# UbiquitousLearning/Mandheling-DSP-Training

Hardware: AMD Instinct MI355X
Metric: training images/sec + int8 MFMA TOPS, VGG-11 batch 256, 1/2/4/8 MI355X (higher is better)
Workload: dtype int8; 1 GPU; VGG11 NITI int8 training step (fwd+relu+pool, loss grad, weight grad, input grad, SGD), 3x32x32; global_batch=256, per_gpu_batch=256, parallelism=single GPU, streams=one stream (weight gradient, then input gradient, per layer)

## Files before the change

include/niti_hip.h:

```cpp
#ifndef NITI_HIP_H
#define NITI_HIP_H

#include <stddef.h>
#include <stdint.h>

#ifdef __cplusplus
extern "C" {
#endif

enum niti_error_code {
    NITI_NO_ERROR = 0,
    NITI_OUT_OF_MEMORY = 1,
    NITI_NOT_SUPPORT = 2,
    NITI_COMPUTE_SIZE_ERROR = 3,
    NITI_NO_EXECUTION = 4,
    NITI_INVALID_VALUE = 5,
    NITI_INPUT_DATA_ERROR = 10,
    NITI_CALL_BACK_STOP = 11
};

enum niti_op_type {
    NITI_OP_CONV_INT8 = 700,
    NITI_OP_DECONV_INT8 = 701,
    NITI_OP_RELU_INT8 = 703,
// ... 85 lines not shown
int niti_conv_fwd_phase1(const niti_geom* g, const int8_t* x_nhwc16, const int8_t* w_ohwi16, int32_t* acc,
                         uint32_t* amax, void* workspace, size_t workspace_bytes, void* stream);
int niti_conv_fwd_phase2(const niti_geom* g, const int8_t* x_nhwc16, const int8_t* w_ohwi16, const int32_t* acc,
                         const uint32_t* amax, const int8_t* exp_in, const int8_t* wscale, int8_t* exp_out, int relu,
                         const int8_t* relu_mask, int8_t* out_nhwc16, size_t workspace_bytes, void* stream);
int niti_conv_dgrad_phase1(const niti_geom* g, const int8_t* dy_nhwc16, const int8_t* wt_ihwo16, int32_t* acc,
                           uint32_t* amax, void* workspace, size_t workspace_bytes, void* stream);
int niti_conv_dgrad_phase2(const niti_geom* g, const int8_t* dy_nhwc16, const int8_t* wt_ihwo16, const int32_t* acc,
                           const uint32_t* amax, const int8_t* exp_in, const int8_t* wscale, int8_t* exp_out,
                           int relu, const int8_t* relu_mask, int8_t* out_nhwc16, size_t workspace_bytes,
                           void* stream);
#define NITI_ROWCONV_STATE_WORDS 1216
uint32_t* niti_rows_spec_slot(uint32_t* state, int dgrad);
int niti_conv_rows_ok(const niti_geom* g);
int niti_conv_rows_plan(const niti_geom* g, int dgrad, int* W, int* R, int* ks, int* workgroups);
int niti_nhwc16_to_c32(const int8_t* in_nhwc16, int n, int hw, int cp, int c, int8_t* out_c32, void* stream);
int niti_weights_to_wf(const int8_t* w_ohwi16, int co, int ci, int cip, int transpose, int8_t* out_wf,
                       void* stream);
#define NITI_ROWS_X_NHWC16 0x100
int niti_conv_rows_nhwc_ok(const niti_geom* g, int flags);
int niti_conv_fwd_rows(const niti_geom* g, const int8_t* x_c32, const int8_t* wf, const int8_t* exp_in,
                       const int8_t* wscale, int8_t* exp_out, int relu, int8_t* out_nhwc16, int8_t* pool_out_nhwc16,
                       int8_t* next_c32, int mode, uint32_t* amax, uint32_t* state, uint32_t epoch, uint32_t* err,
                       void* stream);
int niti_conv_dgrad_rows(const niti_geom* g, const int8_t* dy_c32, const int8_t* wft, const int8_t* relu_mask,
                         const int8_t* pool_x, const int8_t* pool_y, int pool_relu, int8_t* dx_nhwc16, int8_t* dx_c32,
                         int8_t* dx_p16, const int8_t* exp_in, const int8_t* wscale, int8_t* exp_out, int mode,
                         uint32_t* amax, uint32_t* state, uint32_t epoch, uint32_t* err, void* stream);
int niti_conv_wgrad_acc(const niti_geom* g, const int8_t* x_nhwc16, const int8_t* dy_nhwc16, int32_t* acc,
                        uint32_t* amax, void* workspace, size_t workspace_bytes, void* stream);
int niti_nhwc16_to_p16(const int8_t* in_nhwc16, int64_t pixels, int cp, int8_t* out_p16, void* stream);
int niti_conv_wgrad_p16_workspace(const niti_geom* g, int splits, size_t* bytes);
void niti_diag_wgrad_stamps(void* buf);
void niti_diag_rowconv_stamps(void* buf);
void niti_diag_rowconv_barrier(uint32_t spin_limit, uint32_t expect_extra);
void niti_diag_rowconv_speculate(int mode);
void niti_diag_gemm_speculate(int bias);
unsigned long long niti_diag_gemm_fused_launches(void);
unsigned long long niti_diag_head_chain_launches(void);
void niti_diag_head_chain(int on);
void niti_diag_p16_jobs_cap(int cap);
int niti_conv_wgrad_p16_acc(const niti_geom* g, const int8_t* x_p16, const int8_t* dy_p16, int32_t* acc,
                            uint32_t* amax, void* workspace, size_t workspace_bytes, int splits, void* stream);
typedef struct niti_wgrad_p16_job {
    niti_geom g;
    const int8_t* x_p16;
    const int8_t* dy_p16;
    int32_t* acc;
    uint32_t* amax;
} niti_wgrad_p16_job;
int niti_conv_wgrad_p16_many_workspace(const niti_wgrad_p16_job* jobs, int n, int blocks, int t, size_t* bytes);
// ... 282 lines not shown
```

mandheling-dsp-training_amd/csrc/niti_capi.hip:

```cpp
#include "../../include/niti_hip.h"
#include <memory>
#include <vector>

#include "niti_internal.hpp"
#include "niti_kernels.hpp"

struct niti_execution {
    niti::Execution* impl = nullptr;
    int op = 0;
    std::vector<void*> stage;
    std::vector<size_t> stage_bytes;
    uint32_t* err_host = nullptr;
    ~niti_execution() {
        delete impl;
        for (void* p : stage)
            if (p) (void)hipFree(p);
        if (err_host) (void)hipHostFree(err_host);
    }
};

namespace {
int code(hipError_t e) {
    if (e == hipSuccess) return NITI_NO_ERROR;
    if (e == hipErrorOutOfMemory) return NITI_OUT_OF_MEMORY;
// ... 258 lines not shown
    o.exp_in = exp_in;
    o.wscale = wscale;
    o.exp_out = exp_out;
    return o;
}

int niti_conv_rows_ok(const niti_geom* g) {
    niti::ConvGeom r;
    return g && to_geom(g, &r) && niti::rowconv_ok(r) ? 1 : 0;
}

int niti_conv_rows_plan(const niti_geom* g, int dgrad, int* W, int* R, int* ks, int* workgroups) {
    niti::ConvGeom r, d;
    if (!g || !W || !R || !ks || !workgroups || !to_geom(g, &r)) return 0;
    if (dgrad && !niti::rowconv_dgrad_geom(r, &d)) return 0;
    return niti::rowconv_plan(dgrad ? d : r, dgrad != 0, W, R, ks, workgroups) ? 1 : 0;
}

int niti_nhwc16_to_c32(const int8_t* in, int n, int hw, int cp, int c, int8_t* out, void* stream) {
    if (!in || !out || n <= 0 || hw <= 0 || c <= 0 || cp < c || cp % 16) return NITI_INVALID_VALUE;
    return code(niti::nhwc16_to_c32(in, n, hw, cp, c, out, S(stream)));
}

int niti_weights_to_wf(const int8_t* w, int co, int ci, int cip, int transpose, int8_t* out, void* stream) {
    if (!w || !out || co <= 0 || ci <= 0 || cip < ci || cip % 16) return NITI_INVALID_VALUE;
    return code(niti::weights_to_wf(w, co, ci, cip, transpose != 0, out, S(stream)));
}

int niti_conv_rows_nhwc_ok(const niti_geom* g, int dgrad) {
    if (!g) return 0;
    niti::ConvGeom r, d;
    if (!to_geom(g, &r)) return 0;
// ... 29 lines not shown
}

int niti_conv_dgrad_rows(const niti_geom* g, const int8_t* dy_c32, const int8_t* wft, const int8_t* relu_mask,
                         const int8_t* pool_x, const int8_t* pool_y, int pool_relu, int8_t* dx, int8_t* dx_c32,
                         int8_t* dx_p16, const int8_t* exp_in, const int8_t* wscale, int8_t* exp_out, int mode,
                         uint32_t* amax, uint32_t* state, uint32_t epoch, uint32_t* err, void* stream) {
    const int x_nhwc = (mode & NITI_ROWS_X_NHWC16) ? 1 : 0;
    mode &= ~NITI_ROWS_X_NHWC16;
    if (!g || !dy_c32 || !wft || !amax || mode < 0 || mode > 4) return NITI_INVALID_VALUE;
    if (mode >= 3 && state == nullptr) return NITI_INVALID_VALUE;
    if ((pool_x == nullptr) != (pool_y == nullptr) || (pool_x && relu_mask)) return NITI_INVALID_VALUE;
    if (mode != 1 && dx == nullptr) return NITI_INVALID_VALUE;
    niti::ConvGeom r, d;
    if (!to_geom(g, &r)) return NITI_COMPUTE_SIZE_ERROR;
    if (!niti::rowconv_dgrad_geom(r, &d)) return NITI_NOT_SUPPORT;
    if (mode == 0 && !niti::rowconv_fused_ok(d, true)) return NITI_NOT_SUPPORT;
    if (dx_p16 != nullptr && !niti::rowconv_p16_ok(d, pool_x != nullptr)) return NITI_NOT_SUPPORT;
    if (x_nhwc && !niti::rowconv_nhwc_ok(d)) return NITI_NOT_SUPPORT;
    niti::RowConvOut o;
    o.x_nhwc = x_nhwc;
    o.p16 = dx_p16;
    o.exp_in = exp_in;
    o.wscale = wscale;
    o.exp_out = exp_out;
    o.dgrad_slot = 1;
    if (pool_x != nullptr) {
        o.pool_x = pool_x;
        o.pool_y = pool_y;
        o.pool_dx = dx;
        o.pool_dx_next = dx_c32;
        o.pool_relu = pool_relu;
// ... 690 lines not shown
```

mandheling-dsp-training_amd/csrc/niti_kernels.hpp:

```cpp
#pragma once

#include <hip/hip_runtime.h>
#include <stdint.h>
#include <stdlib.h>

#include "../../include/niti_hip.h"

namespace niti {

inline int round_up(int x, int m) { return (x + m - 1) / m * m; }

constexpr int MAX_SLOTS = 64;
constexpr int MAX_SLOT_STRIDE = 32;
constexpr int MAX_WORDS = MAX_SLOTS * MAX_SLOT_STRIDE;
constexpr size_t MAX_BYTES = MAX_WORDS * sizeof(uint32_t);

struct ConvGeom {
    int n, c_in, h, w;
    int c_out, kh, kw;
    int sh, sw, pt, pl, pb, pr, dh, dw;
    int oh, ow;
    int cip, cop, np;
    bool finalize();
};
// ... 217 lines not shown
    int relu = 0;
    const int8_t* relu_mask = nullptr;
    const int8_t* pool_x = nullptr;
    const int8_t* pool_y = nullptr;
    int8_t* pool_dx = nullptr;
    int8_t* pool_dx_next = nullptr;
    int pool_relu = 0;
    const int8_t* pool_code = nullptr;
    int8_t* pool_code_out = nullptr;
    int pool_dx_nhwc = 1;
    int8_t* p16 = nullptr;
    int32_t* acc_store = nullptr;
    int dgrad_slot = 0;
    int x_nhwc = 0;
};
size_t rowconv_acc_bytes(const ConvGeom& g, bool dg);
bool rowconv_nhwc_ok(const ConvGeom& g);
bool rowconv_nhwc_pref(const ConvGeom& g);
constexpr int ROWCONV_BAR_WORDS = 2 * 19 * 32;
static_assert(ROWCONV_BAR_WORDS == NITI_ROWCONV_STATE_WORDS, "header constant");
bool rowconv_ok(const ConvGeom& g);
bool rowconv_seg(const ConvGeom& g);
bool rowconv_dgrad_geom(const ConvGeom& layer, ConvGeom* d);
bool rowconv_p16_ok(const ConvGeom& d, bool pool);
bool rowconv_fused_ok(const ConvGeom& g, bool dg = false);
int rowconv_units(const ConvGeom& g, bool dg = false);
bool rowconv_plan(const ConvGeom& g, bool dg, int* W, int* R, int* ks, int* wgs);
size_t rowconv_wf_bytes(int co, int ci);
hipError_t nhwc16_to_c32(const int8_t* in, int n, int hw, int cp, int c, int8_t* out, hipStream_t st);
hipError_t c32_to_nhwc16(const int8_t* in, int n, int hw, int cp, int c, int8_t* out, hipStream_t st);
hipError_t weights_to_wf(const int8_t* w_ohwi16, int co, int ci, int cip, bool transpose, int8_t* out,
                         hipStream_t st);
constexpr int RC_SPEC_A = 3, RC_SPEC_B = 4;
bool rowconv_spec2_on();
void rowconv_stamps_arm(unsigned long long* buf);
void rowconv_barrier_diag(uint32_t spin_limit, uint32_t expect_extra);
void rowconv_speculate(int mode);
uint32_t* rowconv_spec_slot(uint32_t* bar, bool dg);
void model_p16_jobs_cap(int cap);
void model_wgrad_batch(int mode);
void model_wgrad_quad(int kg);
int wgrad_quad_kg(int own);
// ... 197 lines not shown
```

mandheling-dsp-training_amd/csrc/niti_model.hip:

```cpp
#include <stdlib.h>
#include <string.h>

#include <algorithm>
#include <array>
#include <memory>
#include <vector>

#include "../../include/niti_hip.h"
#include "niti_map.hpp"
#include "niti_step_driver.hpp"

namespace niti {

namespace {
extern int g_p16_jobs_cap;
extern int g_wgrad_batch;
extern int g_wgrad_quad;
extern int g_c0w_mode;
extern unsigned long long g_c0w_launches;
}
void model_p16_jobs_cap(int cap) { g_p16_jobs_cap = cap <= 0 ? P16_MAX_JOBS : cap; }
void model_wgrad_batch(int mode) { g_wgrad_batch = mode < 0 ? 1 : mode; }
void model_wgrad_quad(int kg) { g_wgrad_quad = kg < 0 ? -1 : kg; }
int wgrad_quad_kg(int own) { return g_wgrad_quad >= 0 ? g_wgrad_quad : own; }
// ... 744 lines not shown
        }
        if (!l.col && !l.dw && rowconv_ok(g)) {
            l.rc = 1;
            l.wf = (int8_t*)ws.alloc(rowconv_wf_bytes(g.c_out, g.c_in));
            l.xc32 = (int8_t*)ws.alloc((size_t)n * round_up(g.c_in, 32) * g.h * g.w);
            if (!l.wf || !l.xc32) return NITI_OUT_OF_MEMORY;
            if (hipMemset(l.wf, 0, rowconv_wf_bytes(g.c_out, g.c_in)) != hipSuccess)
                return NITI_NO_EXECUTION;
            rc_acc_size = std::max(rc_acc_size, rowconv_acc_bytes(g, false));
            const Layer* pv = i > 0 ? &L[i - 1] : nullptr;
            const bool pv_ok = pv != nullptr && !pv->flatten && pv->g.cop == g.cip &&
                               (pv->pool ? (pv->ph == g.h && pv->pw == g.w && pv->g.oh == 2 * g.h && pv->g.ow == 2 * g.w)
                                         : (pv->g.oh == g.h && pv->g.ow == g.w));
            if (pv_ok && rowconv_dgrad_geom(g, &l.dg)) {
                l.rcd = 1;
                rc_acc_size = std::max(rc_acc_size, rowconv_acc_bytes(l.dg, true));
                l.wft = (int8_t*)ws.alloc(rowconv_wf_bytes(g.c_in, g.c_out));
                l.dyc32 = (int8_t*)ws.alloc(out_px * round_up(g.c_out, 32));
                if (!l.wft || !l.dyc32) return NITI_OUT_OF_MEMORY;
                if (hipMemset(l.wft, 0, rowconv_wf_bytes(g.c_in, g.c_out)) != hipSuccess) return NITI_NO_EXECUTION;
            }
        }
        if (!l.dw && conv_wgrad_p16_ok(g)) {
            slab_w_bytes = std::max(slab_w_bytes, conv_wgrad_p16_workspace(g, 8));
            xp16[i] = (int8_t*)ws.alloc((size_t)n * g.h * g.w * g.cip);
            l.slab16_bytes = conv_wgrad_p16_workspace(g, 8);
            l.slab16 = l.slab16_bytes ? (int32_t*)ws.alloc(l.slab16_bytes) : nullptr;
            if (l.slab16_bytes && !l.slab16) return NITI_OUT_OF_MEMORY;
            dp16[i] = (int8_t*)ws.alloc(out_px * g.cop);
            if (!xp16[i] || !dp16[i]) return NITI_OUT_OF_MEMORY;
        }
// ... 355 lines not shown
            } else {
                o.pool_x = pv.r;
                o.pool_y = pv.p;
            }
            o.pool_dx = pv.dy;
            o.pool_dx_next = next;
            o.pool_relu = pv.relu;
            o.pool_dx_nhwc = skip16 ? 0 : 1;
        } else {
            o.out = skip16 ? nullptr : pv.dy;
            o.next = next;
            o.relu_mask = pv.relu ? pv.r : nullptr;
        }
        dy16_valid[i - 1] = !skip16 && !g0_only;
        const bool dgk = !g0_only;
        const int rc = rowconv_ranged(rowconv_fused_ok(d, dgk), rowconv_acc_bytes(d, dgk) != 0, o, rng(i, 1), l.bar,
                                      l.epoch, st,
                                      [&](const RowConvOut& ro, int mode, uint32_t* bar, uint32_t epoch, uint32_t* err) {
                                          return rowconv_fwd(d, dyin, l.wft, ro, mode, rng(i, 1), bar, epoch, err, st);
                                      });
        if (rc != NITI_NO_ERROR) return rc;
        probe(i, 1, false, st);
        dp16_valid[i - 1] = o.p16 != nullptr ? 1 : 0;
        dyc32_valid[i - 1] = next != nullptr ? 1 : 0;
        return NITI_NO_ERROR;
    }
    dy16_valid[i - 1] = 1;
    const ConvGeom& pg = pv.g;
    const bool sub = l.subw != nullptr;
    const bool spec = !l.dw && conv_dgrad_spec_ok(g);
    int8_t* p16_out = !l.dw && !sub && !spec && fuse_dp16 && wgrad_p16_splits(i - 1) > 0 ? dp16[i - 1] : nullptr;
// ... 787 lines not shown
```

mandheling-dsp-training_amd/csrc/niti_rowconv.hip:

```cpp
#include <hip/hip_runtime.h>

#include <stdlib.h>

#include <algorithm>
#include <map>
#include <mutex>

#include "niti_device.hpp"
#include "niti_gridbar.hpp"
#include "niti_kernels.hpp"
#include "niti_map.hpp"

#ifndef RC_EXP
#define RC_EXP 0
#endif
namespace niti {

__device__ __forceinline__ int bitwidth_rc(uint32_t m) { return m <= 1u ? 0 : 32 - __clz((int)(m - 1u)); }

__device__ __forceinline__ int32_t psto_rc(int32_t a, int s) {
    const uint32_t ua = a < 0 ? 0u - (uint32_t)a : (uint32_t)a;
    const uint32_t q = ua >> s;
    const uint32_t prob = ua & ((1u << s) - 1u);
    const int h = s >> 1;
// ... 137 lines not shown
constexpr int RC_LDS_BYTES = RC_MAX_STAGES * RC_STAGE_BYTES;
constexpr int RC_P16_WAVE_BYTES = 16 * 1024;
constexpr int RC_SMEM_BYTES = RC_LDS_BYTES > 4 * RC_P16_WAVE_BYTES ? RC_LDS_BYTES : 4 * RC_P16_WAVE_BYTES;
constexpr int RC_KS_MAX_NS = 4;
constexpr int RC_KS_BYTES = 4 * RC_KS_MAX_NS * 9 * 1024;
static_assert(RC_KS_BYTES >= 4 * RC_P16_WAVE_BYTES, "the P16 tile fits the K-split ring");

template <int W, int R, bool UNC>
__device__ __forceinline__ void rowconv_compute(const RowConvArgs& a, const RowUnit<W, R>& U, int lane, int wid,
                                                int8_t* smem, v16i (&acc)[R]) {
    constexpr int NR = R + 2, WS = W == 0 ? 16 : W;
    const int H = W == 0 ? a.hw : W, WR = W == 0 ? a.hw : W;
    constexpr bool DPPX = true;
    constexpr int KXL = DPPX ? 1 : 3;
    constexpr int S = 4;
    constexpr int L = KXL * NR + 3;
    const int h = lane >> 5, c = lane & 31, ox = W == 0 ? U.x : c % WS;
    const __amdgpu_buffer_rsrc_t rX = make_rsrc(a.x, a.xbytes);
    const __amdgpu_buffer_rsrc_t rW = make_rsrc(a.wf, a.wbytes);
    const uint32_t xl = !(U.img_ok && U.x_ok) ? OOB
                        : W == 0 ? (uint32_t)U.img * a.xis + (uint32_t)ox * a.xps + 16u * h
                                 : (uint32_t)((((int64_t)U.img * a.CB * H) * WR + ox) * 32 + 16 * h);
    const uint32_t CHUNK = W == 0 ? a.xcs : (uint32_t)H * WR * 32;
    const uint32_t XROW = W == 0 ? a.xrs : (uint32_t)WR * 32;
    const int y0 = U.b * R - 1;
#pragma unroll
    for (int r = 0; r < R; ++r)
#pragma unroll
        for (int i = 0; i < 16; ++i) acc[r][i] = 0;
    uint32_t off[3][NR];
#pragma unroll
    for (int j = 0; j < NR; ++j) {
        const int iy = y0 + j;
        const bool row_ok = iy >= 0 && iy < H && xl != OOB;
        const uint32_t base = xl + (uint32_t)iy * XROW;
        off[0][j] = row_ok && ox > 0 ? base - 32u : OOB;
        off[1][j] = row_ok ? base : OOB;
        off[2][j] = row_ok && ox < WR - 1 ? base + 32u : OOB;
    }
    const uint32_t dv2 = wid == 0 ? (uint32_t)lane * 16u : OOB;
    const int cb = a.CB;
    constexpr bool ONE_BLOCK = W != 0;
    const uint32_t wbase =
        (uint32_t)(ONE_BLOCK ? __builtin_amdgcn_readfirstlane(U.cob * cb * 9) : U.cob * cb * 9) * 1024u;
    v4i X[S][KXL][NR];
    auto issue = [&](auto st_c, int cc) {
        constexpr int ST = decltype(st_c)::value;
        int8_t* lds = smem + ST * RC_STAGE_BYTES;
#pragma unroll
        for (int k = 0; k < 3; ++k) {
            const int piece = wid + 4 * k;
            dma16(rW, lds + piece * 1024, k < 2 ? (uint32_t)lane * 16u : dv2,
                  wbase + (uint32_t)cc * 9216u + (uint32_t)(piece < 9 ? piece : 0) * 1024u);
        }
#pragma unroll
        for (int j = 0; j < NR; ++j)
#pragma unroll
            for (int kx = 0; kx < KXL; ++kx)
                X[ST][kx][j] = buf_load16(rX, off[DPPX ? 1 : kx][j] + (uint32_t)cc * CHUNK);
    };
    const uint32_t lds_lane = lds_addr(smem) + (uint32_t)lane * 16u;
    unsigned long long t_wait = 0, t_read = 0, t_issue = 0;
    const bool stamp = a.stamps != nullptr;
    v4i wreg[2][9];
    auto read_w = [&](auto st_c, v4i (&w)[9]) {
        constexpr int ST = decltype(st_c)::value;
#pragma unroll
        for (int t = 0; t < 9; ++t) w[t] = lds_b128(lds_lane + (uint32_t)(ST * RC_STAGE_BYTES + t * 1024));
    };
    auto fence_w = [&](v4i (&w)[9]) {
        asm volatile("s_waitcnt lgkmcnt(0)" ::: "memory");
#pragma unroll
        for (int t = 0; t < 9; ++t) reg_fence(w[t]);
    };
    auto arrive = [&](int later) {
        if (later >= 1)
            asm volatile("s_waitcnt vmcnt(%0)" ::"n"(L) : "memory");
        else
            asm volatile("s_waitcnt vmcnt(0)" ::: "memory");
        __builtin_amdgcn_s_barrier();
        asm volatile("" ::: "memory");
    };
    constexpr bool SKIP = W > 0 && R == W && !(RC_EXP & 32);
// ... 13 lines not shown
            }
        if (more && !(RC_EXP & 4)) read_w(std::integral_constant<int, (ST + 1) % S>(), wreg[1 - WB]);
        const v4i (&w)[9] = wreg[(RC_EXP & 4) ? 0 : WB];
        if constexpr (DPPX) {
            v4i XL[NR], XR[NR];
            auto taps = [&](int j) {
                XL[j] = (RC_EXP & 1) ? X[ST][0][j] : shift_in_left<WS>(X[ST][0][j], ox == 0);
                XR[j] = (RC_EXP & 1) ? X[ST][0][j] : shift_in_right<WS>(X[ST][0][j], ox == WS - 1);
            };
            auto mfma3 = [&](int r, int ky) {
                acc[r] = __builtin_amdgcn_mfma_i32_32x32x32_i8(w[3 * ky], XL[r + ky], acc[r], 0, 0, 0);
                acc[r] = __builtin_amdgcn_mfma_i32_32x32x32_i8(w[3 * ky + 1], X[ST][0][r + ky], acc[r], 0, 0, 0);
                acc[r] = __builtin_amdgcn_mfma_i32_32x32x32_i8(w[3 * ky + 2], XR[r + ky], acc[r], 0, 0, 0);
            };
#pragma unroll
            for (int j = SKIP ? 1 : 0; j < (SKIP ? NR - 1 : NR); ++j) taps(j);
#pragma unroll
            for (int r = 0; r < R; ++r)
#pragma unroll
                for (int ky = SKIP && r == 0 ? 1 : 0; ky < (SKIP && r == R - 1 ? 2 : 3); ++ky) mfma3(r, ky);
        } else {
#pragma unroll
            for (int r = 0; r < R; ++r)
#pragma unroll
                for (int ky = 0; ky < 3; ++ky)
#pragma unroll
                    for (int kx = 0; kx < 3; ++kx)
                        acc[r] = __builtin_amdgcn_mfma_i32_32x32x32_i8(w[3 * ky + kx], X[ST][kx][r + ky], acc[r], 0, 0, 0);
        }
        if constexpr (ONE_BLOCK) {
            if (more) fence_w(wreg[1 - WB]);
        } else {
            const unsigned long long s2 = stamp ? __builtin_amdgcn_s_memtime() : 0ull;
            if (more) fence_w(wreg[1 - WB]);
            if (stamp) {
// ... 18 lines not shown
            step(std::integral_constant<int, 0>(), cc);
            step(std::integral_constant<int, 1>(), cc + 1);
            step(std::integral_constant<int, 2>(), cc + 2);
            step(std::integral_constant<int, 3>(), cc + 3);
        }
        asm volatile("s_waitcnt vmcnt(0)" ::: "memory");
    } else {
        for (int cc = 0; cc < cb; cc += S) {
            step(std::integral_constant<int, 0>(), cc);
            if (cc + 1 < cb) step(std::integral_constant<int, 1>(), cc + 1);
            if (cc + 2 < cb) step(std::integral_constant<int, 2>(), cc + 2);
            if (cc + 3 < cb) step(std::integral_constant<int, 3>(), cc + 3);
        }
    }
    __builtin_amdgcn_s_barrier();
    if (stamp && lane == 0) {
        unsigned long long* st = a.stamps + (blockIdx.x * 4 + wid) * 16;
        st[3] = __builtin_amdgcn_s_memtime();
        st[2] = t_issue;
        st[6] = t_wait;
        st[7] = t_read;
    }
}

template <int W, int R, int NS>
__device__ __forceinline__ void rowconv_compute_ks(const RowConvArgs& a, const RowUnit<W, R>& U, int lane, int wid,
                                                   int8_t* smem, v16i (&acc)[R]) {
    static_assert(R == W && NS >= 1 && NS <= RC_KS_MAX_NS, "whole-image units, all chunks staged at once");
    constexpr int H = W;
    const int h = lane >> 5, c = lane & 31, ox = c % W;
// ... 1076 lines not shown
    static const int v = getenv("NITI_RC_ACC_MIN_CIN") ? atoi(getenv("NITI_RC_ACC_MIN_CIN")) : 256;
    return v;
}
static bool seg_store_acc(const ConvGeom& g) { return g.c_in >= acc_min_cin(); }

bool rowconv_dgrad_geom(const ConvGeom& l, ConvGeom* d) {
    if (!rowconv_ok(l)) return false;
    ConvGeom g = l;
    g.c_in = l.c_out;
    g.c_out = l.c_in;
    if (!g.finalize() || g.cip != l.cop || g.cop != l.cip) return false;
    *d = g;
    return rowconv_ok(g);
}

static int rowconv_rows(const ConvGeom& g, bool dg, int* units_out) {
    if (rowconv_seg(g)) {
        const SegPlan p = seg_plan(g);
        *units_out = p.wgs * 4;
        return p.R;
    }
    const int W = g.w, G = 32 / W;
    const int64_t groups = (g.n + G - 1) / G, cob = g.cop / 32;
    int R = W == 16 && !dg ? 8 : (W < 4 ? W : 4);
    if (RC_EXP & 16) R = 2;
    while (R > 2 && groups * (W / R) * cob < 768) R /= 2;
    const int64_t ngb4 = (groups * (W / R) + 3) / 4 * 4;
    *units_out = (int)(ngb4 * cob);
    return R;
}

static int rowconv_ks(const ConvGeom& g, bool dg);

size_t rowconv_acc_bytes(const ConvGeom& g, bool dg) {
    if (!rowconv_ok(g)) return 0;
    if (rowconv_seg(g)) {
        const SegPlan p = seg_plan(g);
        return seg_store_acc(g) ? (size_t)p.wgs * 4 * p.R * 1024 * sizeof(int32_t) : 0;
    }
    if (getenv("NITI_RC_ACC_MIN_CIN") != nullptr && g.c_in < acc_min_cin()) return 0;
    int u = 0;
    const int R = rowconv_rows(g, dg, &u);
    const int G = 32 / g.w, ngb = ((g.n + G - 1) / G) * (g.h / R), ngb4 = (ngb + 3) / 4 * 4, COB = g.cop / 32;
    const int64_t wgs = rowconv_ks(g, dg) > 0 ? (int64_t)COB * ngb : (int64_t)COB * ngb4 / 4;
    return (size_t)wgs * 4 * R * 1024 * sizeof(int32_t);
}

bool rowconv_p16_ok(const ConvGeom& d, bool pool) {
    if (!rowconv_ok(d) || rowconv_seg(d)) return false;
    int u = 0;
    const int R = rowconv_rows(d, true, &u), W = d.w;
    const int64_t px = (int64_t)d.n * d.h * d.w * (pool ? 4 : 1);
    if (px % 16 != 0) return false;
    return pool || R * W >= 16 || (W == 2 && R == 2) || (W == 4 && R == 2);
}

static int rowconv_ks(const ConvGeom& g, bool dg) {
    int u = 0;
    const int R = rowconv_rows(g, dg, &u);
    const int CB = (g.c_in + 31) / 32;
    if (g.w != 2 || R != 2 || CB % 4 != 0 || CB / 4 > RC_KS_MAX_NS || u >= 768) return 0;
    return CB / 4;
}

int rowconv_units(const ConvGeom& g, bool dg) {
    if (rowconv_seg(g)) return seg_plan(g).wgs * 4;
    int u = 0;
    (void)rowconv_rows(g, dg, &u);
    if (rowconv_ks(g, dg) > 0) {
        const int64_t units = (int64_t)(g.n + 15) / 16 * (g.cop / 32);
        return (int)(units * 4);
    }
    return u;
}

template <int MODE, bool DG>
static const void* rc_kernel(int W, int R, bool unc, int ks) {
    if constexpr (MODE == RC_REQUANT && DG) {
        if (W == 0 && ks == 1 && R == 4) return reinterpret_cast<const void*>(&rowconv_fwd_kernel<0, 4, MODE, DG, false, 1>);
        if (W == 0 && ks == 1 && R == 2) return reinterpret_cast<const void*>(&rowconv_fwd_kernel<0, 2, MODE, DG, false, 1>);
    }
    if (W == 0 && ks != 0) return nullptr;
    if (ks > 0) {
        if (ks == 4) return reinterpret_cast<const void*>(&rowconv_fwd_kernel<2, 2, MODE, DG, false, 4>);
        if (ks == 2) return reinterpret_cast<const void*>(&rowconv_fwd_kernel<2, 2, MODE, DG, false, 2>);
        if (ks == 1) return reinterpret_cast<const void*>(&rowconv_fwd_kernel<2, 2, MODE, DG, false, 1>);
        return nullptr;
    }
#define RC_CASE(WW, RR)                                                                                  \
    if (W == WW && R == RR)                                                                              \
        return (WW != 1 && unc) ? reinterpret_cast<const void*>(&rowconv_fwd_kernel<WW, RR, MODE, DG, true, 0>) \
                                : reinterpret_cast<const void*>(&rowconv_fwd_kernel<WW, RR, MODE, DG, false, 0>);
    if constexpr (!DG) RC_CASE(16, 8)
    RC_CASE(16, 4)
    RC_CASE(16, 2)
    RC_CASE(8, 4)
    RC_CASE(8, 2)
    RC_CASE(4, 4)
    RC_CASE(4, 2)
    RC_CASE(2, 2)
    RC_CASE(1, 1)
    RC_CASE(0, 4)
    RC_CASE(0, 2)
#undef RC_CASE
    return nullptr;
}

template <int MODE, bool DG>
static hipError_t launch_rc(int W, int R, int grid, RowConvArgs a, hipStream_t st, int ks = 0) {
    const void* f = rc_kernel<MODE, DG>(W, R, W != 1 && a.CB % 4 == 0, ks);
    if (f == nullptr) return hipErrorInvalidValue;
    void* args[] = {&a};
    return hipLaunchKernel(f, dim3((unsigned)grid), dim3(256), args, 0, st);
}
// ... 7 lines not shown
        return 0;
    }
    std::lock_guard<std::mutex> lk(mu);
    const auto key = std::make_pair(dev, f);
    auto it = cache.find(key);
    if (it != cache.end()) return it->second;
    int cus = 0, occ = 0;
    if (hipDeviceGetAttribute(&cus, hipDeviceAttributeMultiprocessorCount, dev) != hipSuccess ||
        hipOccupancyMaxActiveBlocksPerMultiprocessor(&occ, f, threads, 0) != hipSuccess) {
        (void)hipGetLastError();
        return 0;
    }
    return cache[key] = cus * occ;
}

static int rowconv_wgs(const ConvGeom& g, bool dg, int* R_out, int* ks_out) {
    if (rowconv_seg(g)) {
        const SegPlan p = seg_plan(g);
        *R_out = p.R;
        *ks_out = 0;
        return p.wgs;
    }
    int u = 0;
    const int R = rowconv_rows(g, dg, &u);
    const int ks = rowconv_ks(g, dg);
    const int G = 32 / g.w, ngb = ((g.n + G - 1) / G) * (g.h / R), ngb4 = (ngb + 3) / 4 * 4, COB = g.cop / 32;
    *R_out = R;
    *ks_out = ks;
    return ks > 0 ? COB * ngb : COB * ngb4 / 4;
}

bool rowconv_plan(const ConvGeom& g, bool dg, int* W, int* R, int* ks, int* wgs) {
    if (!rowconv_ok(g)) return false;
    *wgs = rowconv_wgs(g, dg, R, ks);
    *W = rowconv_seg(g) ? 0 : g.w;
    return true;
}

bool rowconv_fused_ok(const ConvGeom& g, bool dg) {
    if (!rowconv_ok(g)) return false;
    int R = 0, ks = 0;
    const int wgs = rowconv_wgs(g, dg, &R, &ks);
    const bool unc = (g.c_in + 31) / 32 % 4 == 0;
    const int W = rowconv_seg(g) ? 0 : g.w;
    const void* f = dg ? rc_kernel<RC_FUSED, true>(W, R, unc, ks) : rc_kernel<RC_FUSED, false>(W, R, unc, ks);
    return wgs <= resident_wgs(f);
}

static uint32_t g_rc_spin_limit = BAR_SPIN_LIMIT, g_rc_expect_extra = 0;
static int g_rc_spec = 0;
void rowconv_barrier_diag(uint32_t spin_limit, uint32_t expect_extra) {
    g_rc_spin_limit = spin_limit ? spin_limit : BAR_SPIN_LIMIT;
    g_rc_expect_extra = expect_extra;
}
void rowconv_speculate(int mode) { g_rc_spec = mode; }
uint32_t* rowconv_spec_slot(uint32_t* bar, bool dg) { return bar + (16 + (dg ? 1 : 0)) * BAR_LINE; }
static bool spec_scale_on() {
// ... 48 lines not shown
        a.xcs = 32u;
    } else {
        a.xps = 32u;
        a.xrs = (uint32_t)(g.w * 32);
        a.xis = (uint32_t)(CB * g.h * g.w * 32);
        a.xcs = (uint32_t)(g.h * g.w * 32);
    }
    a.x = x_c32;
    a.wf = wf;
    a.xbytes = (uint32_t)xb;
    a.wbytes = (uint32_t)wb;
    a.n = g.n;
    a.CB = CB;
    a.COB = COB;
    const bool dg = o.relu_mask != nullptr || o.pool_dx != nullptr || o.p16 != nullptr;
    int units = 0;
    const int R = rowconv_rows(g, dg, &units);
    const bool seg = rowconv_seg(g);
    const int Wk = seg ? 0 : g.w;
    int ks = 0;
    if (seg) {
        const SegPlan p = seg_plan(g);
        a.hw = g.w;
        a.gw = p.gw;
        a.nsp = p.nsp;
        a.nbands = p.nbands;
        a.ngb = p.ngb;
        a.upc4 = p.upc4;
        a.wgs = p.wgs;
    } else {
        const int G = 32 / g.w;
        a.nbands = g.h / R;
        a.ngb = ((g.n + G - 1) / G) * a.nbands;
        a.ngb4 = (a.ngb + 3) / 4 * 4;
        ks = rowconv_ks(g, dg);
        a.wgs = ks > 0 ? COB * a.ngb : COB * a.ngb4 / 4;
    }
    a.wmajor = rowconv_wmajor(xb, wb);
    a.out = o.out;
    a.cop = g.cop;
    a.pool_out = o.pool_out;
    a.next = o.next;
    a.exp_in = o.exp_in;
    a.wscale = o.wscale;
    a.exp_out = o.exp_out;
    a.relu = o.relu;
    a.amax = amax;
    a.bar = bar;
    a.epoch = epoch;
    a.err = err;
// ... 8 lines not shown
    a.pool_dx_next = o.pool_dx_next;
    a.pool_relu = o.pool_relu;
    a.pool_code = o.pool_code;
    a.pool_code_out = o.pool_code_out;
    a.pool_dx_nhwc = o.pool_dx_nhwc;
    a.p16 = o.p16;
    a.p16_pixels = (int64_t)g.n * g.h * g.w * (o.pool_dx != nullptr ? 4 : 1);
    a.acc_store = mode == RC_FUSED ? nullptr : o.acc_store;
    a.spec2 = spec2;
    a.spec_cooldown = spec_cooldown();
    a.hint = (spec || mode == RC_FUSED) && bar != nullptr ? bar + (16 + (dg || o.dgrad_slot ? 1 : 0)) * BAR_LINE : nullptr;
    a.hint_scale = dg || o.dgrad_slot || !spec_scale_on() ? 0 : 1;
    if (o.p16 != nullptr && (!dg || !rowconv_p16_ok(g, o.pool_dx != nullptr))) return hipErrorInvalidValue;
    if (o.pool_out != nullptr && (R % 2 != 0 || g.h % 2 != 0)) return hipErrorInvalidValue;
    if (mode == RC_FUSED) {
        if (bar == nullptr || err == nullptr || epoch == 0 || !rowconv_fused_ok(g, dg)) return hipErrorInvalidValue;
        return dg ? launch_rc<RC_FUSED, true>(Wk, R, a.wgs, a, st, ks) : launch_rc<RC_FUSED, false>(Wk, R, a.wgs, a, st, ks);
    }
    int grid = a.wgs;
    grid = grid > 1024 ? 1024 : grid;
    if (seg) {
        ks = mode == RC_REQUANT && dg && o.pool_dx != nullptr ? 1 : 0;
        const void* f = mode == RC_RANGE ? rc_kernel<RC_RANGE, false>(0, R, false, 0)
                                         : (dg ? rc_kernel<RC_REQUANT, true>(0, R, false, ks)
                                               : rc_kernel<RC_REQUANT, false>(0, R, false, 0));
        const int res = resident_wgs(f);
        if (res > 0 && grid > res) grid = res;
    }
    if (mode == RC_RANGE) return launch_rc<RC_RANGE, false>(Wk, R, grid, a, st, ks);
    return dg ? launch_rc<RC_REQUANT, true>(Wk, R, grid, a, st, ks) : launch_rc<RC_REQUANT, false>(Wk, R, grid, a, st, ks);
}
// ... 142 lines not shown
```

mandheling-dsp-training_amd/niti_amd/_lib.py:

```python
from __future__ import annotations

import ctypes as C
import os
import re

_HERE = os.path.dirname(os.path.abspath(__file__))
LIB_PATH = os.environ.get("NITI_HIP_LIB") or os.path.join(_HERE, "_lib", "libniti_hip.so")
HEADER = os.path.join(os.path.dirname(os.path.dirname(_HERE)), "include", "niti_hip.h")

ERROR_NAMES = {0: "NO_ERROR", 1: "OUT_OF_MEMORY", 2: "NOT_SUPPORT", 3: "COMPUTE_SIZE_ERROR",
               4: "NO_EXECUTION", 5: "INVALID_VALUE", 10: "INPUT_DATA_ERROR", 11: "CALL_BACK_STOP"}
NOT_SUPPORT, INVALID_VALUE = 2, 5

OP_CONV_INT8 = 700
OP_DECONV_INT8 = 701
OP_RELU_INT8 = 703
OP_RELUGRAD_INT8 = 704
OP_MAXPOOL_INT8 = 705
OP_POOLGRAD_INT8 = 706
OP_LOSS_INT8 = 710
OP_LOSS_GRAD_INT8 = 711
OP_MATMUL_INT8 = 713
OP_PAD_INT8 = 714
OP_LEFTPOOLGRAD_INT8 = 718
# ... 122 lines not shown
                          f"make -C mandheling-dsp-training_amd/csrc")
    import torch
    L = C.CDLL(LIB_PATH)
    vp, i32, i64, ci = C.c_void_p, C.c_int32, C.c_int64, C.c_int
    tp = C.POINTER(Tensor)
    sig = {
        "niti_version": (C.c_char_p, []),
        "niti_create_execution": (ci, [ci, C.POINTER(ConvCommon), C.POINTER(vp)]),
        "niti_execution_resize": (ci, [vp, tp, ci, tp, ci]),
        "niti_execution_execute": (ci, [vp, tp, ci, tp, ci, vp]),
        "niti_destroy_execution": (None, [vp]),
        "niti_execution_workspace_bytes": (C.c_size_t, [vp]),
        "niti_execution_status": (ci, [vp, vp]),
        "niti_diag_rowconv_barrier": (None, [C.c_uint32, C.c_uint32]),
        "niti_diag_rowconv_speculate": (None, [C.c_int]),
        "niti_diag_gemm_speculate": (None, [C.c_int]),
        "niti_diag_gemm_fused_launches": (C.c_ulonglong, []),
        "niti_diag_head_chain_launches": (C.c_ulonglong, []),
        "niti_diag_head_chain": (None, [C.c_int]),
        "niti_diag_p16_jobs_cap": (None, [C.c_int]),
        "niti_diag_wgrad_batch": (None, [C.c_int]),
        "niti_diag_wgrad_batch_launches": (C.c_ulonglong, []),
        "niti_diag_wgrad_quad": (None, [C.c_int]),
        "niti_conv_wgrad_p16_many_items": (ci, [C.POINTER(WgradP16Job), ci, ci, ci, C.POINTER(ci), ci, C.POINTER(ci),
                                                ci, C.POINTER(ci)]),
        "niti_tensor_convert": (ci, [tp, tp, vp]),
        "niti_geom_finalize": (ci, [C.POINTER(Geom)]),
        "niti_conv_workspace_bytes": (ci, [C.POINTER(Geom), ci, C.POINTER(C.c_size_t)]),
        "niti_matmul_workspace_bytes": (ci, [ci, ci, ci, C.POINTER(C.c_size_t)]),
        "niti_conv_plan_info": (ci, [C.POINTER(Geom), ci, C.c_size_t, C.POINTER(C.c_int)]),
        "niti_conv_fwd_acc": (ci, [C.POINTER(Geom), vp, vp, vp, vp, vp, C.c_size_t, vp]),
        "niti_conv_dgrad_acc": (ci, [C.POINTER(Geom), vp, vp, vp, vp, vp, C.c_size_t, vp]),
        "niti_conv_wgrad_acc": (ci, [C.POINTER(Geom), vp, vp, vp, vp, vp, C.c_size_t, vp]),
        "niti_conv_fwd_phase1": (ci, [C.POINTER(Geom), vp, vp, vp, vp, vp, C.c_size_t, vp]),
        "niti_conv_rows_ok": (ci, [C.POINTER(Geom)]),
        "niti_conv_rows_plan": (ci, [C.POINTER(Geom), ci, C.POINTER(ci), C.POINTER(ci), C.POINTER(ci), C.POINTER(ci)]),
        "niti_nhwc16_to_c32": (ci, [vp, ci, ci, ci, ci, vp, vp]),
        "niti_weights_to_wf": (ci, [vp, ci, ci, ci, ci, vp, vp]),
        "niti_conv_fwd_rows": (ci, [C.POINTER(Geom), vp, vp, vp, vp, vp, ci, vp, vp, vp, ci, vp, vp, C.c_uint32, vp,
                                    vp]),
        "niti_conv_dgrad_rows": (ci, [C.POINTER(Geom), vp, vp, vp, vp, vp, ci, vp, vp, vp, vp, vp, vp, ci, vp, vp, C.c_uint32, vp, vp]),
        "niti_rows_spec_slot": (vp, [vp, ci]),
        "niti_conv_fwd_phase2": (ci, [C.POINTER(Geom), vp, vp, vp, vp, vp, vp, vp, ci, vp, vp, C.c_size_t, vp]),
        "niti_conv_dgrad_phase1": (ci, [C.POINTER(Geom), vp, vp, vp, vp, vp, C.c_size_t, vp]),
        "niti_conv_dgrad_phase2": (ci, [C.POINTER(Geom), vp, vp, vp, vp, vp, vp, vp, ci, vp, vp, C.c_size_t, vp]),
        "niti_nhwc16_to_p16": (ci, [vp, i64, ci, vp, vp]),
        "niti_diag_wgrad_stamps": (None, [vp]),
        "niti_diag_rowconv_stamps": (None, [vp]),
        "niti_conv_wgrad_p16_workspace": (ci, [C.POINTER(Geom), ci, C.POINTER(C.c_size_t)]),
        "niti_conv_wgrad_p16_acc": (ci, [C.POINTER(Geom), vp, vp, vp, vp, vp, C.c_size_t, ci, vp]),
        "niti_conv_wgrad_p16_many_workspace": (ci, [C.POINTER(WgradP16Job), ci, ci, ci, C.POINTER(C.c_size_t)]),
# ... 138 lines not shown
```

mandheling-dsp-training_amd/niti_amd/ops.py:

```python
from __future__ import annotations

import ctypes as C

import torch

from . import _lib as L
from ._lib import check


def _stream(stream=None):
    if stream is not None:
        return stream
    return C.c_void_p(torch.cuda.current_stream().cuda_stream)


def _ptr(t):
    return None if t is None else C.c_void_p(t.data_ptr())


def tensor(t: torch.Tensor, dims, fmt=L.FORMAT_NCHW) -> L.Tensor:
    d = list(dims) + [1] * (4 - len(dims))
    v = L.Tensor(t.data_ptr(), (C.c_int * 4)(*d), fmt)
    v._keep = t
    return v
# ... 160 lines not shown
    check(p1(C.byref(g), _ptr(a), _ptr(b), _ptr(acc), _ptr(amax), _ptr(ws), nb, _stream(stream)), "conv phase 1")
    if between is not None:
        between(amax)
    check(p2(C.byref(g), _ptr(a), _ptr(b), _ptr(acc), _ptr(amax), _ptr(exp_in), _ptr(wscale), _ptr(exp_out),
             1 if relu else 0, _ptr(relu_mask), _ptr(out), nb, _stream(stream)), "conv phase 2")
    return out


ROWCONV_STATE_WORDS = 1216


def conv_rows_ok(g: L.Geom) -> bool:
    return bool(L.lib().niti_conv_rows_ok(C.byref(g)))


def conv_rows_plan(g: L.Geom, dgrad=False):
    w, r, ks, wgs = C.c_int(), C.c_int(), C.c_int(), C.c_int()
    if not L.lib().niti_conv_rows_plan(C.byref(g), 1 if dgrad else 0, C.byref(w), C.byref(r), C.byref(ks),
                                       C.byref(wgs)):
        return None
    return w.value, r.value, ks.value, wgs.value


def nhwc16_to_c32(x16: torch.Tensor, c: int, stream=None, out=None):
    n, h, w, cp = x16.shape
    cb = (c + 31) // 32
    if out is None:
        out = torch.empty((n, cb, h, w, 32), dtype=torch.int8, device=x16.device)
    check(L.lib().niti_nhwc16_to_c32(_ptr(x16), n, h * w, cp, c, _ptr(out), _stream(stream)), "nhwc16->c32")
    return out


def weights_to_wf(w16: torch.Tensor, ci: int, transpose=False, stream=None, out=None):
    co, cip = w16.shape[0], w16.shape[-1]
# ... 616 lines not shown
```

Measured before the change: 812,800 images/s.

## Use one-row bands with mirrored halo loads for pooled 4-wide dgrad rowconv

For pooled input-gradient convolutions at width 4, the row planner now picks one output row per band (R=1) instead of two when the unit count falls in a mid range, raising parallelism. A MIRROR variant of the row-conv kernel (W == 2R) lets the second band flip its row order and swap ky weight slices, so both bands skip the top halo row load and its MFMAs, and the accumulators are swapped back afterwards. This adds a new kernel instantiation and a pooled flag threaded through the planning functions, plus an env/diag toggle. It risks more workgroups and lower per-workgroup weight reuse.

```diff
diff --git a/include/niti_hip.h b/include/niti_hip.h
--- a/include/niti_hip.h
+++ b/include/niti_hip.h
@@ -123,6 +123,7 @@
 uint32_t* niti_rows_spec_slot(uint32_t* state, int dgrad);
 int niti_conv_rows_ok(const niti_geom* g);
 int niti_conv_rows_plan(const niti_geom* g, int dgrad, int* W, int* R, int* ks, int* workgroups);
+int niti_conv_rows_plan2(const niti_geom* g, int dgrad, int pooled, int* W, int* R, int* ks, int* workgroups);
 int niti_nhwc16_to_c32(const int8_t* in_nhwc16, int n, int hw, int cp, int c, int8_t* out_c32, void* stream);
 int niti_weights_to_wf(const int8_t* w_ohwi16, int co, int ci, int cip, int transpose, int8_t* out_wf,
                        void* stream);
@@ -144,6 +145,7 @@
 void niti_diag_rowconv_stamps(void* buf);
 void niti_diag_rowconv_barrier(uint32_t spin_limit, uint32_t expect_extra);
 void niti_diag_rowconv_speculate(int mode);
+void niti_diag_rowconv_rows1(int mode);
 void niti_diag_gemm_speculate(int bias);
 unsigned long long niti_diag_gemm_fused_launches(void);
 unsigned long long niti_diag_head_chain_launches(void);
diff --git a/mandheling-dsp-training_amd/csrc/niti_capi.hip b/mandheling-dsp-training_amd/csrc/niti_capi.hip
--- a/mandheling-dsp-training_amd/csrc/niti_capi.hip
+++ b/mandheling-dsp-training_amd/csrc/niti_capi.hip
@@ -296,8 +296,17 @@
     niti::ConvGeom r, d;
     if (!g || !W || !R || !ks || !workgroups || !to_geom(g, &r)) return 0;
     if (dgrad && !niti::rowconv_dgrad_geom(r, &d)) return 0;
-    return niti::rowconv_plan(dgrad ? d : r, dgrad != 0, W, R, ks, workgroups) ? 1 : 0;
-}
+    return niti::rowconv_plan(dgrad ? d : r, dgrad != 0, false, W, R, ks, workgroups) ? 1 : 0;
+}
+
+int niti_conv_rows_plan2(const niti_geom* g, int dgrad, int pooled, int* W, int* R, int* ks, int* workgroups) {
+    niti::ConvGeom r, d;
+    if (!g || !W || !R || !ks || !workgroups || !to_geom(g, &r)) return 0;
+    if (dgrad && !niti::rowconv_dgrad_geom(r, &d)) return 0;
+    return niti::rowconv_plan(dgrad ? d : r, dgrad != 0, dgrad != 0 && pooled != 0, W, R, ks, workgroups) ? 1 : 0;
+}
+
+void niti_diag_rowconv_rows1(int mode) { niti::rowconv_rows1(mode); }
 
 int niti_nhwc16_to_c32(const int8_t* in, int n, int hw, int cp, int c, int8_t* out, void* stream) {
     if (!in || !out || n <= 0 || hw <= 0 || c <= 0 || cp < c || cp % 16) return NITI_INVALID_VALUE;
@@ -357,7 +366,7 @@
     niti::ConvGeom r, d;
     if (!to_geom(g, &r)) return NITI_COMPUTE_SIZE_ERROR;
     if (!niti::rowconv_dgrad_geom(r, &d)) return NITI_NOT_SUPPORT;
-    if (mode == 0 && !niti::rowconv_fused_ok(d, true)) return NITI_NOT_SUPPORT;
+    if (mode == 0 && !niti::rowconv_fused_ok(d, true, pool_x != nullptr)) return NITI_NOT_SUPPORT;
     if (dx_p16 != nullptr && !niti::rowconv_p16_ok(d, pool_x != nullptr)) return NITI_NOT_SUPPORT;
     if (x_nhwc && !niti::rowconv_nhwc_ok(d)) return NITI_NOT_SUPPORT;
     niti::RowConvOut o;
diff --git a/mandheling-dsp-training_amd/csrc/niti_kernels.hpp b/mandheling-dsp-training_amd/csrc/niti_kernels.hpp
--- a/mandheling-dsp-training_amd/csrc/niti_kernels.hpp
+++ b/mandheling-dsp-training_amd/csrc/niti_kernels.hpp
@@ -255,7 +255,7 @@
     int dgrad_slot = 0;
     int x_nhwc = 0;
 };
-size_t rowconv_acc_bytes(const ConvGeom& g, bool dg);
+size_t rowconv_acc_bytes(const ConvGeom& g, bool dg, bool pooled = false);
 bool rowconv_nhwc_ok(const ConvGeom& g);
 bool rowconv_nhwc_pref(const ConvGeom& g);
 constexpr int ROWCONV_BAR_WORDS = 2 * 19 * 32;
@@ -264,9 +264,10 @@
 bool rowconv_seg(const ConvGeom& g);
 bool rowconv_dgrad_geom(const ConvGeom& layer, ConvGeom* d);
 bool rowconv_p16_ok(const ConvGeom& d, bool pool);
-bool rowconv_fused_ok(const ConvGeom& g, bool dg = false);
-int rowconv_units(const ConvGeom& g, bool dg = false);
-bool rowconv_plan(const ConvGeom& g, bool dg, int* W, int* R, int* ks, int* wgs);
+bool rowconv_fused_ok(const ConvGeom& g, bool dg = false, bool pooled = false);
+int rowconv_units(const ConvGeom& g, bool dg = false, bool pooled = false);
+bool rowconv_plan(const ConvGeom& g, bool dg, bool pooled, int* W, int* R, int* ks, int* wgs);
+void rowconv_rows1(int mode);
 size_t rowconv_wf_bytes(int co, int ci);
 hipError_t nhwc16_to_c32(const int8_t* in, int n, int hw, int cp, int c, int8_t* out, hipStream_t st);
 hipError_t c32_to_nhwc16(const int8_t* in, int n, int hw, int cp, int c, int8_t* out, hipStream_t st);
diff --git a/mandheling-dsp-training_amd/csrc/niti_model.hip b/mandheling-dsp-training_amd/csrc/niti_model.hip
--- a/mandheling-dsp-training_amd/csrc/niti_model.hip
+++ b/mandheling-dsp-training_amd/csrc/niti_model.hip
@@ -782,7 +782,7 @@
                                          : (pv->g.oh == g.h && pv->g.ow == g.w));
             if (pv_ok && rowconv_dgrad_geom(g, &l.dg)) {
                 l.rcd = 1;
-                rc_acc_size = std::max(rc_acc_size, rowconv_acc_bytes(l.dg, true));
+                rc_acc_size = std::max(rc_acc_size, rowconv_acc_bytes(l.dg, true, pv->pool != 0));
                 l.wft = (int8_t*)ws.alloc(rowconv_wf_bytes(g.c_in, g.c_out));
                 l.dyc32 = (int8_t*)ws.alloc(out_px * round_up(g.c_out, 32));
                 if (!l.wft || !l.dyc32) return NITI_OUT_OF_MEMORY;
@@ -1168,7 +1168,8 @@
         }
         dy16_valid[i - 1] = !skip16 && !g0_only;
         const bool dgk = !g0_only;
-        const int rc = rowconv_ranged(rowconv_fused_ok(d, dgk), rowconv_acc_bytes(d, dgk) != 0, o, rng(i, 1), l.bar,
+        const bool pooled = o.pool_dx != nullptr;
+        const int rc = rowconv_ranged(rowconv_fused_ok(d, dgk, pooled), rowconv_acc_bytes(d, dgk, pooled) != 0, o, rng(i, 1), l.bar,
                                       l.epoch, st,
                                       [&](const RowConvOut& ro, int mode, uint32_t* bar, uint32_t epoch, uint32_t* err) {
                                           return rowconv_fwd(d, dyin, l.wft, ro, mode, rng(i, 1), bar, epoch, err, st);
diff --git a/mandheling-dsp-training_amd/csrc/niti_rowconv.hip b/mandheling-dsp-training_amd/csrc/niti_rowconv.hip
--- a/mandheling-dsp-training_amd/csrc/niti_rowconv.hip
+++ b/mandheling-dsp-training_amd/csrc/niti_rowconv.hip
@@ -175,7 +175,9 @@
     constexpr bool DPPX = true;
     constexpr int KXL = DPPX ? 1 : 3;
     constexpr int S = 4;
-    constexpr int L = KXL * NR + 3;
+    constexpr bool MIRROR = W > 0 && W == 2 * R && !(RC_EXP & 64);
+    constexpr int J0 = MIRROR ? 1 : 0;
+    constexpr int L = KXL * (NR - J0) + 3;
     const int h = lane >> 5, c = lane & 31, ox = W == 0 ? U.x : c % WS;
     const __amdgpu_buffer_rsrc_t rX = make_rsrc(a.x, a.xbytes);
     const __amdgpu_buffer_rsrc_t rW = make_rsrc(a.wf, a.wbytes);
@@ -185,6 +187,7 @@
     const uint32_t CHUNK = W == 0 ? a.xcs : (uint32_t)H * WR * 32;
     const uint32_t XROW = W == 0 ? a.xrs : (uint32_t)WR * 32;
     const int y0 = U.b * R - 1;
+    const bool flip = MIRROR && __builtin_amdgcn_readfirstlane(U.b) == 1;
 #pragma unroll
     for (int r = 0; r < R; ++r)
 #pragma unroll
@@ -192,7 +195,7 @@
     uint32_t off[3][NR];
 #pragma unroll
     for (int j = 0; j < NR; ++j) {
-        const int iy = y0 + j;
+        const int iy = flip ? H - j : y0 + j;
         const bool row_ok = iy >= 0 && iy < H && xl != OOB;
         const uint32_t base = xl + (uint32_t)iy * XROW;
         off[0][j] = row_ok && ox > 0 ? base - 32u : OOB;
@@ -215,19 +218,26 @@
                   wbase + (uint32_t)cc * 9216u + (uint32_t)(piece < 9 ? piece : 0) * 1024u);
         }
 #pragma unroll
-        for (int j = 0; j < NR; ++j)
+        for (int j = J0; j < NR; ++j)
 #pragma unroll
             for (int kx = 0; kx < KXL; ++kx)
                 X[ST][kx][j] = buf_load16(rX, off[DPPX ? 1 : kx][j] + (uint32_t)cc * CHUNK);
     };
     const uint32_t lds_lane = lds_addr(smem) + (uint32_t)lane * 16u;
+    const uint32_t lds_ky0 = lds_lane + (flip ? 6u * 1024u : 0u), lds_ky2 = lds_lane + (flip ? 0u : 6u * 1024u);
     unsigned long long t_wait = 0, t_read = 0, t_issue = 0;
     const bool stamp = a.stamps != nullptr;
     v4i wreg[2][9];
     auto read_w = [&](auto st_c, v4i (&w)[9]) {
         constexpr int ST = decltype(st_c)::value;
 #pragma unroll
-        for (int t = 0; t < 9; ++t) w[t] = lds_b128(lds_lane + (uint32_t)(ST * RC_STAGE_BYTES + t * 1024));
+        for (int t = 0; t < 9; ++t) {
+            if constexpr (MIRROR)
+                w[t] = lds_b128((t < 3 ? lds_ky0 : (t < 6 ? lds_lane : lds_ky2)) +
+                                (uint32_t)(ST * RC_STAGE_BYTES + (t < 6 ? t : t - 6) * 1024));
+            else
+                w[t] = lds_b128(lds_lane + (uint32_t)(ST * RC_STAGE_BYTES + t * 1024));
+        }
     };
     auto fence_w = [&](v4i (&w)[9]) {
         asm volatile("s_waitcnt lgkmcnt(0)" ::: "memory");
@@ -271,11 +281,11 @@
                 acc[r] = __builtin_amdgcn_mfma_i32_32x32x32_i8(w[3 * ky + 2], XR[r + ky], acc[r], 0, 0, 0);
             };
 #pragma unroll
-            for (int j = SKIP ? 1 : 0; j < (SKIP ? NR - 1 : NR); ++j) taps(j);
+            for (int j = SKIP || MIRROR ? 1 : 0; j < (SKIP ? NR - 1 : NR); ++j) taps(j);
 #pragma unroll
             for (int r = 0; r < R; ++r)
 #pragma unroll
-                for (int ky = SKIP && r == 0 ? 1 : 0; ky < (SKIP && r == R - 1 ? 2 : 3); ++ky) mfma3(r, ky);
+                for (int ky = (SKIP || MIRROR) && r == 0 ? 1 : 0; ky < (SKIP && r == R - 1 ? 2 : 3); ++ky) mfma3(r, ky);
         } else {
 #pragma unroll
             for (int r = 0; r < R; ++r)
@@ -324,6 +334,16 @@
         }
     }
     __builtin_amdgcn_s_barrier();
+    if constexpr (MIRROR) {
+        if (flip) {
+#pragma unroll
+            for (int r = 0; r < R / 2; ++r) {
+                const v16i t = acc[r];
+                acc[r] = acc[R - 1 - r];
+                acc[R - 1 - r] = t;
+            }
+        }
+    }
     if (stamp && lane == 0) {
         unsigned long long* st = a.stamps + (blockIdx.x * 4 + wid) * 16;
         st[3] = __builtin_amdgcn_s_memtime();
@@ -1430,7 +1450,13 @@
     return rowconv_ok(g);
 }
 
-static int rowconv_rows(const ConvGeom& g, bool dg, int* units_out) {
+static int g_rc_rows1 = -1;
+void rowconv_rows1(int mode) { g_rc_rows1 = mode < 0 ? -1 : (mode != 0 ? 1 : 0); }
+static bool rows1_on() {
+    static const bool env = getenv("NITI_RC_ROWS1") ? atoi(getenv("NITI_RC_ROWS1")) != 0 : true;
+    return g_rc_rows1 < 0 ? env : g_rc_rows1 != 0;
+}
+static int rowconv_rows(const ConvGeom& g, bool dg, bool pooled, int* units_out) {
     if (rowconv_seg(g)) {
         const SegPlan p = seg_plan(g);
         *units_out = p.wgs * 4;
@@ -1441,14 +1467,18 @@
     int R = W == 16 && !dg ? 8 : (W < 4 ? W : 4);
     if (RC_EXP & 16) R = 2;
     while (R > 2 && groups * (W / R) * cob < 768) R /= 2;
+    if (dg && pooled && W == 4 && R == 2 && rows1_on()) {
+        const int64_t u2 = groups * 2 * cob;
+        if (u2 >= 384 && u2 <= 512) R = 1;
+    }
     const int64_t ngb4 = (groups * (W / R) + 3) / 4 * 4;
     *units_out = (int)(ngb4 * cob);
     return R;
 }
 
-static int rowconv_ks(const ConvGeom& g, bool dg);
-
-size_t rowconv_acc_bytes(const ConvGeom& g, bool dg) {
+static int rowconv_ks(const ConvGeom& g, bool dg, bool pooled);
+
+size_t rowconv_acc_bytes(const ConvGeom& g, bool dg, bool pooled) {
     if (!rowconv_ok(g)) return 0;
     if (rowconv_seg(g)) {
         const SegPlan p = seg_plan(g);
@@ -1456,34 +1486,34 @@
     }
     if (getenv("NITI_RC_ACC_MIN_CIN") != nullptr && g.c_in < acc_min_cin()) return 0;
     int u = 0;
-    const int R = rowconv_rows(g, dg, &u);
+    const int R = rowconv_rows(g, dg, pooled, &u);
     const int G = 32 / g.w, ngb = ((g.n + G - 1) / G) * (g.h / R), ngb4 = (ngb + 3) / 4 * 4, COB = g.cop / 32;
-    const int64_t wgs = rowconv_ks(g, dg) > 0 ? (int64_t)COB * ngb : (int64_t)COB * ngb4 / 4;
+    const int64_t wgs = rowconv_ks(g, dg, pooled) > 0 ? (int64_t)COB * ngb : (int64_t)COB * ngb4 / 4;
     return (size_t)wgs * 4 * R * 1024 * sizeof(int32_t);
 }
 
 bool rowconv_p16_ok(const ConvGeom& d, bool pool) {
     if (!rowconv_ok(d) || rowconv_seg(d)) return false;
     int u = 0;
-    const int R = rowconv_rows(d, true, &u), W = d.w;
+    const int R = rowconv_rows(d, true, pool, &u), W = d.w;
     const int64_t px = (int64_t)d.n * d.h * d.w * (pool ? 4 : 1);
     if (px % 16 != 0) return false;
     return pool || R * W >= 16 || (W == 2 && R == 2) || (W == 4 && R == 2);
 }
 
-static int rowconv_ks(const ConvGeom& g, bool dg) {
+static int rowconv_ks(const ConvGeom& g, bool dg, bool pooled) {
     int u = 0;
-    const int R = rowconv_rows(g, dg, &u);
+    const int R = rowconv_rows(g, dg, pooled, &u);
     const int CB = (g.c_in + 31) / 32;
     if (g.w != 2 || R != 2 || CB % 4 != 0 || CB / 4 > RC_KS_MAX_NS || u >= 768) return 0;
     return CB / 4;
 }
 
-int rowconv_units(const ConvGeom& g, bool dg) {
+int rowconv_units(const ConvGeom& g, bool dg, bool pooled) {
     if (rowconv_seg(g)) return seg_plan(g).wgs * 4;
     int u = 0;
-    (void)rowconv_rows(g, dg, &u);
-    if (rowconv_ks(g, dg) > 0) {
+    (void)rowconv_rows(g, dg, pooled, &u);
+    if (rowconv_ks(g, dg, pooled) > 0) {
         const int64_t units = (int64_t)(g.n + 15) / 16 * (g.cop / 32);
         return (int)(units * 4);
     }
@@ -1514,6 +1544,7 @@
     RC_CASE(8, 2)
     RC_CASE(4, 4)
     RC_CASE(4, 2)
+    if constexpr (DG || MODE == RC_RANGE) RC_CASE(4, 1)
     RC_CASE(2, 2)
     RC_CASE(1, 1)
     RC_CASE(0, 4)
@@ -1551,7 +1582,7 @@
     return cache[key] = cus * occ;
 }
 
-static int rowconv_wgs(const ConvGeom& g, bool dg, int* R_out, int* ks_out) {
+static int rowconv_wgs(const ConvGeom& g, bool dg, bool pooled, int* R_out, int* ks_out) {
     if (rowconv_seg(g)) {
         const SegPlan p = seg_plan(g);
         *R_out = p.R;
@@ -1559,25 +1590,25 @@
         return p.wgs;
     }
     int u = 0;
-    const int R = rowconv_rows(g, dg, &u);
-    const int ks = rowconv_ks(g, dg);
+    const int R = rowconv_rows(g, dg, pooled, &u);
+    const int ks = rowconv_ks(g, dg, pooled);
     const int G = 32 / g.w, ngb = ((g.n + G - 1) / G) * (g.h / R), ngb4 = (ngb + 3) / 4 * 4, COB = g.cop / 32;
     *R_out = R;
     *ks_out = ks;
     return ks > 0 ? COB * ngb : COB * ngb4 / 4;
 }
 
-bool rowconv_plan(const ConvGeom& g, bool dg, int* W, int* R, int* ks, int* wgs) {
+bool rowconv_plan(const ConvGeom& g, bool dg, bool pooled, int* W, int* R, int* ks, int* wgs) {
     if (!rowconv_ok(g)) return false;
-    *wgs = rowconv_wgs(g, dg, R, ks);
+    *wgs = rowconv_wgs(g, dg, pooled, R, ks);
     *W = rowconv_seg(g) ? 0 : g.w;
     return true;
 }
 
-bool rowconv_fused_ok(const ConvGeom& g, bool dg) {
+bool rowconv_fused_ok(const ConvGeom& g, bool dg, bool pooled) {
     if (!rowconv_ok(g)) return false;
     int R = 0, ks = 0;
-    const int wgs = rowconv_wgs(g, dg, &R, &ks);
+    const int wgs = rowconv_wgs(g, dg, pooled, &R, &ks);
     const bool unc = (g.c_in + 31) / 32 % 4 == 0;
     const int W = rowconv_seg(g) ? 0 : g.w;
     const void* f = dg ? rc_kernel<RC_FUSED, true>(W, R, unc, ks) : rc_kernel<RC_FUSED, false>(W, R, unc, ks);
@@ -1656,8 +1687,9 @@
     a.CB = CB;
     a.COB = COB;
     const bool dg = o.relu_mask != nullptr || o.pool_dx != nullptr || o.p16 != nullptr;
+    const bool pooled = o.pool_dx != nullptr;
     int units = 0;
-    const int R = rowconv_rows(g, dg, &units);
+    const int R = rowconv_rows(g, dg, pooled, &units);
     const bool seg = rowconv_seg(g);
     const int Wk = seg ? 0 : g.w;
     int ks = 0;
@@ -1675,7 +1707,7 @@
         a.nbands = g.h / R;
         a.ngb = ((g.n + G - 1) / G) * a.nbands;
         a.ngb4 = (a.ngb + 3) / 4 * 4;
-        ks = rowconv_ks(g, dg);
+        ks = rowconv_ks(g, dg, pooled);
         a.wgs = ks > 0 ? COB * a.ngb : COB * a.ngb4 / 4;
     }
     a.wmajor = rowconv_wmajor(xb, wb);
@@ -1714,7 +1746,7 @@
     if (o.p16 != nullptr && (!dg || !rowconv_p16_ok(g, o.pool_dx != nullptr))) return hipErrorInvalidValue;
     if (o.pool_out != nullptr && (R % 2 != 0 || g.h % 2 != 0)) return hipErrorInvalidValue;
     if (mode == RC_FUSED) {
-        if (bar == nullptr || err == nullptr || epoch == 0 || !rowconv_fused_ok(g, dg)) return hipErrorInvalidValue;
+        if (bar == nullptr || err == nullptr || epoch == 0 || !rowconv_fused_ok(g, dg, pooled)) return hipErrorInvalidValue;
         return dg ? launch_rc<RC_FUSED, true>(Wk, R, a.wgs, a, st, ks) : launch_rc<RC_FUSED, false>(Wk, R, a.wgs, a, st, ks);
     }
     int grid = a.wgs;
diff --git a/mandheling-dsp-training_amd/niti_amd/_lib.py b/mandheling-dsp-training_amd/niti_amd/_lib.py
--- a/mandheling-dsp-training_amd/niti_amd/_lib.py
+++ b/mandheling-dsp-training_amd/niti_amd/_lib.py
@@ -160,6 +160,7 @@
         "niti_execution_status": (ci, [vp, vp]),
         "niti_diag_rowconv_barrier": (None, [C.c_uint32, C.c_uint32]),
         "niti_diag_rowconv_speculate": (None, [C.c_int]),
+        "niti_diag_rowconv_rows1": (None, [C.c_int]),
         "niti_diag_gemm_speculate": (None, [C.c_int]),
         "niti_diag_gemm_fused_launches": (C.c_ulonglong, []),
         "niti_diag_head_chain_launches": (C.c_ulonglong, []),
@@ -181,6 +182,8 @@
         "niti_conv_fwd_phase1": (ci, [C.POINTER(Geom), vp, vp, vp, vp, vp, C.c_size_t, vp]),
         "niti_conv_rows_ok": (ci, [C.POINTER(Geom)]),
         "niti_conv_rows_plan": (ci, [C.POINTER(Geom), ci, C.POINTER(ci), C.POINTER(ci), C.POINTER(ci), C.POINTER(ci)]),
+        "niti_conv_rows_plan2": (ci, [C.POINTER(Geom), ci, ci, C.POINTER(ci), C.POINTER(ci), C.POINTER(ci),
+                                      C.POINTER(ci)]),
         "niti_nhwc16_to_c32": (ci, [vp, ci, ci, ci, ci, vp, vp]),
         "niti_weights_to_wf": (ci, [vp, ci, ci, ci, ci, vp, vp]),
         "niti_conv_fwd_rows": (ci, [C.POINTER(Geom), vp, vp, vp, vp, vp, ci, vp, vp, vp, ci, vp, vp, C.c_uint32, vp,
diff --git a/mandheling-dsp-training_amd/niti_amd/ops.py b/mandheling-dsp-training_amd/niti_amd/ops.py
--- a/mandheling-dsp-training_amd/niti_amd/ops.py
+++ b/mandheling-dsp-training_amd/niti_amd/ops.py
@@ -198,10 +198,15 @@
     return bool(L.lib().niti_conv_rows_ok(C.byref(g)))
 
 
-def conv_rows_plan(g: L.Geom, dgrad=False):
+def conv_rows_plan(g: L.Geom, dgrad=False, pooled=False):
     w, r, ks, wgs = C.c_int(), C.c_int(), C.c_int(), C.c_int()
-    if not L.lib().niti_conv_rows_plan(C.byref(g), 1 if dgrad else 0, C.byref(w), C.byref(r), C.byref(ks),
-                                       C.byref(wgs)):
+    if pooled:
+        ok = L.lib().niti_conv_rows_plan2(C.byref(g), 1 if dgrad else 0, 1, C.byref(w), C.byref(r), C.byref(ks),
+                                          C.byref(wgs))
+    else:
+        ok = L.lib().niti_conv_rows_plan(C.byref(g), 1 if dgrad else 0, C.byref(w), C.byref(r), C.byref(ks),
+                                         C.byref(wgs))
+    if not ok:
         return None
     return w.value, r.value, ks.value, wgs.value
 
```

Result: faster. 821,200 images/s (median of 6 runs) (+1.0%).
